# eth-ait/MultiPly

Hardware: NVIDIA H100
Metric: rays/sec (higher is better)
Workload: dtype f32 (fp16 hi/lo split tensor-core operands, fp32 accumulate)

## Files before the change

multiply_b200/csrc/mlp_tc.cu:

```cuda
#include "common.cuh"
#include <vector>
#include <mutex>
#include <type_traits>
#include <stdlib.h>

namespace mp {

enum {
  K_SP_PLAIN = 0,
  K_SP_SAVE = 1,
  K_SP_SEED = 2,
  K_FEAT = 3,
  K_BWD = 4,
  K_FINAL_GRAD = 5,
  K_RELU = 6
};
enum {
  F_INJECT_EMB = 1,
  F_SDF_DOT = 2,
  F_SKIP_GRAD = 4,
  F_EXTRA_IN = 8,
  F_RGB_OUT = 16
};
constexpr int kMaxSteps = 24;
constexpr int kSlotBytes = 32768;
constexpr int kRing = 3;

struct TcStep {
  int nk;
  int kind;
  int flags;
  int sig;
  const float* bias;
  int slot_off;
  int sc;
  int terms;
};

struct TcProgram {
  int nsteps;
  TcStep step[kMaxSteps];
  const uint4* blob;
  const float* inv_scale;
  int d_in, multires, E, inj_col, n_extra;
  const float* w8row;
  const float* b8;
  const float* Wrgb;
  const float* brgb;
};

struct TcIO : MlpCall {
  float rz;
  char* scratch;
  size_t scratch_per_cta;
  unsigned long long* stalls;
};

constexpr int kConsumers = 2;
constexpr int kThreads = 128 * (1 + kConsumers);

enum { PH_STEP = 0, PH_FULL = 1, PH_WGMMA = 2, PH_BAR = 3, PH_EPI = 4, PH_EMPTY = 5 };
constexpr int kStallWarps = 1 + 4 * kConsumers;
static_assert(MP_STALL_WARPS == kStallWarps && MP_STALL_KINDS == K_RELU + 1 && MP_STALL_PHASES == PH_EMPTY + 1 &&
                  MP_STALL_PROLOGUE == MP_STALL_KINDS * MP_STALL_PHASES && MP_STALL_ELAPSED == MP_STALL_PROLOGUE + 1 &&
                  MP_STALL_WORDS == MP_STALL_ELAPSED + 1,
              "stall record layout of include/multiply_b200.h");
template <bool PROF>
__device__ __forceinline__ long long stall_clock() {
  if constexpr (PROF) return clock64();
  else return 0;
}
__device__ __forceinline__ void stall_add(unsigned long long* rec, int word, long long clocks) {
  atomicAdd(rec + word, (unsigned long long)clocks);
}

constexpr size_t kSigBytes = (size_t)8 * kConsumers * 32 * 128 * 16;
constexpr size_t kFeatBytes = (size_t)kConsumers * 32 * 128 * 16;
constexpr size_t kGeBytes = (size_t)96 * 128 * 4;
constexpr size_t kEmbBytes = (size_t)96 * 128 * 4;
constexpr size_t kScratchPerCta = kSigBytes + kFeatBytes + kGeBytes + kEmbBytes;

constexpr int kAhead = 4;

constexpr int kABytes = 2 * 4 * 128 * 128;
constexpr int kSmemBytes = kABytes + kRing * kSlotBytes + 256 + 1024;
static_assert(kSmemBytes <= 232448, "shared memory budget of one CTA (227 KB)");

__device__ __forceinline__ uint32_t smem_u32(const void* p) { return (uint32_t)__cvta_generic_to_shared(p); }

__device__ __forceinline__ void mbar_init(uint64_t* bar, uint32_t count) {
  asm volatile("mbarrier.init.shared::cta.b64 [%0], %1;" ::"r"(smem_u32(bar)), "r"(count));
}
__device__ __forceinline__ void mbar_arrive(uint64_t* bar) {
  asm volatile("mbarrier.arrive.shared::cta.b64 _, [%0];" ::"r"(smem_u32(bar)) : "memory");
}
__device__ __forceinline__ void mbar_expect_tx(uint64_t* bar, uint32_t bytes) {
  asm volatile("mbarrier.arrive.expect_tx.shared::cta.b64 _, [%0], %1;" ::"r"(smem_u32(bar)), "r"(bytes) : "memory");
}
__device__ __forceinline__ void mbar_wait(uint64_t* bar, uint32_t parity) {
  asm volatile(
      "{\n"
      ".reg .pred p;\n"
      "WAIT_LOOP:\n"
      "mbarrier.try_wait.parity.shared::cta.b64 p, [%0], %1;\n"
      "@p bra WAIT_DONE;\n"
      "bra WAIT_LOOP;\n"
      "WAIT_DONE:\n"
      "}\n" ::"r"(smem_u32(bar)),
      "r"(parity)
      : "memory");
}
__device__ __forceinline__ void bulk_g2s(void* dst, const void* src, uint32_t bytes, uint64_t* bar) {
  asm volatile("cp.async.bulk.shared::cluster.global.mbarrier::complete_tx::bytes [%0], [%1], %2, [%3];" ::"r"(
                   smem_u32(dst)),
               "l"(src), "r"(bytes), "r"(smem_u32(bar))
               : "memory");
}
__device__ __forceinline__ void prefetch_l2(const void* p, uint32_t bytes) {
  asm volatile("cp.async.bulk.prefetch.L2.global [%0], %1;" ::"l"(p), "r"(bytes) : "memory");
}
__device__ __forceinline__ void fence_async_smem() { asm volatile("fence.proxy.async.shared::cta;" ::: "memory"); }

__device__ __forceinline__ void wg_sync(int id) { asm volatile("bar.sync %0, 128;" ::"r"(id) : "memory"); }

__device__ __forceinline__ void wgmma_fence() { asm volatile("wgmma.fence.sync.aligned;" ::: "memory"); }
__device__ __forceinline__ void wgmma_commit() { asm volatile("wgmma.commit_group.sync.aligned;" ::: "memory"); }
template <int N>
__device__ __forceinline__ void wgmma_wait() {
  asm volatile("wgmma.wait_group.sync.aligned %0;" ::"n"(N) : "memory");
}
__device__ __forceinline__ void acc_fence(float* d) {
#pragma unroll
  for (int i = 0; i < 128; ++i) asm volatile("" : "+f"(d[i])::"memory");
}

#define MP_D4(i) "+f"(d[i]), "+f"(d[i + 1]), "+f"(d[i + 2]), "+f"(d[i + 3])
#define MP_D16(i) MP_D4(i), MP_D4(i + 4), MP_D4(i + 8), MP_D4(i + 12)
__device__ __forceinline__ void wgmma_f16(float* d, uint64_t a_desc, uint64_t b_desc, uint32_t accumulate) {
  asm volatile(
      "{\n"
      ".reg .pred p;\n"
      "setp.ne.b32 p, %130, 0;\n"
      "wgmma.mma_async.sync.aligned.m64n256k16.f32.f16.f16 "
      "{%0, %1, %2, %3, %4, %5, %6, %7, %8, %9, %10, %11, %12, %13, %14, %15, "
      "%16, %17, %18, %19, %20, %21, %22, %23, %24, %25, %26, %27, %28, %29, %30, %31, "
      "%32, %33, %34, %35, %36, %37, %38, %39, %40, %41, %42, %43, %44, %45, %46, %47, "
      "%48, %49, %50, %51, %52, %53, %54, %55, %56, %57, %58, %59, %60, %61, %62, %63, "
      "%64, %65, %66, %67, %68, %69, %70, %71, %72, %73, %74, %75, %76, %77, %78, %79, "
      "%80, %81, %82, %83, %84, %85, %86, %87, %88, %89, %90, %91, %92, %93, %94, %95, "
      "%96, %97, %98, %99, %100, %101, %102, %103, %104, %105, %106, %107, %108, %109, %110, %111, "
      "%112, %113, %114, %115, %116, %117, %118, %119, %120, %121, %122, %123, %124, %125, %126, %127}, "
      "%128, %129, p, 1, 1, 0, 0;\n"
      "}\n"
      : MP_D16(0), MP_D16(16), MP_D16(32), MP_D16(48), MP_D16(64), MP_D16(80), MP_D16(96), MP_D16(112)
      : "l"(a_desc), "l"(b_desc), "r"(accumulate));
}
#undef MP_D16
#undef MP_D4

__device__ __forceinline__ uint64_t make_desc(uint32_t saddr) {
  return (uint64_t)((saddr >> 4) & 0x3FFF) | (1ull << 16) | ((uint64_t)(1024 >> 4) << 32) | (1ull << 62);
}

__device__ __forceinline__ uint32_t a_off(int row, int kb, int ch) {
  return (uint32_t)(kb * 16384 + row * 128 + ((ch ^ (row & 7)) << 4));
}

__device__ __forceinline__ void split2(float a, float b, uint32_t& hi, uint32_t& lo) {
  __half2 h = __floats2half2_rn(a, b);
  float2 f = __half22float2(h);
  __half2 l = __floats2half2_rn(a - f.x, b - f.y);
  hi = *(uint32_t*)&h;
  lo = *(uint32_t*)&l;
}
__device__ __forceinline__ void split8(const float* v, uint4& hi, uint4& lo) {
  split2(v[0], v[1], hi.x, lo.x);
  split2(v[2], v[3], hi.y, lo.y);
  split2(v[4], v[5], hi.z, lo.z);
  split2(v[6], v[7], hi.w, lo.w);
}

__device__ __forceinline__ void sts128(uint32_t A32, uint32_t off, const uint4& v) {
  asm volatile("st.shared.v4.b32 [%0], {%1, %2, %3, %4};" ::"r"(A32 + off), "r"(v.x), "r"(v.y), "r"(v.z), "r"(v.w));
}
__device__ __forceinline__ void store_a8(uint32_t A32, int row, int col, const float* v) {
  uint4 hi, lo;
  split8(v, hi, lo);
  uint32_t o = a_off(row, col >> 6, (col >> 3) & 7);
  sts128(A32, o, hi);
  sts128(A32, 65536 + o, lo);
}
__device__ __forceinline__ void stsm4(uint32_t addr, uint32_t a, uint32_t b, uint32_t c, uint32_t e) {
  asm volatile("stmatrix.sync.aligned.m8n8.x4.shared.b16 [%0], {%1, %2, %3, %4};" ::"r"(addr), "r"(a), "r"(b), "r"(c),
               "r"(e));
}
__device__ __forceinline__ void store_pairs(uint32_t lane_base, uint32_t lane_x, int jp, const uint4& hi, const uint4& lo) {
  const uint32_t addr = lane_base + (uint32_t)(jp >> 2) * 16384u + ((((uint32_t)(2 * jp) & 7u) ^ lane_x) << 4);
  stsm4(addr, hi.x, hi.y, hi.z, hi.w);
  stsm4(addr + 65536u, lo.x, lo.y, lo.z, lo.w);
}
__device__ __forceinline__ void store_acc16(uint32_t lane_base, uint32_t lane_x, int jp, const float* v) {
  uint4 hi, lo;
  split8(v, hi, lo);
  store_pairs(lane_base, lane_x, jp, hi, lo);
}

__device__ __forceinline__ float quad_sum(float v) {
  v += __shfl_xor_sync(0xffffffffu, v, 1);
  v += __shfl_xor_sync(0xffffffffu, v, 2);
  return v;
}

__device__ __forceinline__ float4 ld_stream(const float4* p) {
  float4 v;
  asm volatile("ld.global.cg.v4.f32 {%0,%1,%2,%3}, [%4];" : "=f"(v.x), "=f"(v.y), "=f"(v.z), "=f"(v.w) : "l"(p));
  return v;
}
__device__ __forceinline__ uint4 ld_stream(const uint4* p) {
  uint4 v;
  asm volatile("ld.global.cg.v4.u32 {%0,%1,%2,%3}, [%4];" : "=r"(v.x), "=r"(v.y), "=r"(v.z), "=r"(v.w) : "l"(p));
  return v;
}
__device__ __forceinline__ void st_stream(float4* p, const float4& v) {
  asm volatile("st.global.cg.v4.f32 [%0], {%1,%2,%3,%4};" ::"l"(p), "f"(v.x), "f"(v.y), "f"(v.z), "f"(v.w) : "memory");
}
__device__ __forceinline__ void st_stream(uint4* p, const uint4& v) {
  asm volatile("st.global.cg.v4.u32 [%0], {%1,%2,%3,%4};" ::"l"(p), "r"(v.x), "r"(v.y), "r"(v.z), "r"(v.w) : "memory");
}

__device__ __forceinline__ void discard_line(const void* p, float dep) {
  asm volatile("discard.global.L2 [%0], 128;" ::"l"(p), "f"(dep) : "memory");
}
__device__ __forceinline__ void discard_line(const void* p, uint32_t dep) {
  asm volatile("discard.global.L2 [%0], 128;" ::"l"(p), "r"(dep) : "memory");
}

__device__ __forceinline__ float ex2_approx(float x) {
  float y;
  asm("ex2.approx.ftz.f32 %0, %1;" : "=f"(y) : "f"(x));
  return y;
}
__device__ __forceinline__ float lg2_approx(float x) {
  float y;
  asm("lg2.approx.ftz.f32 %0, %1;" : "=f"(y) : "f"(x));
  return y;
}
__device__ __forceinline__ float rcp_approx(float x) {
  float y;
  asm("rcp.approx.ftz.f32 %0, %1;" : "=f"(y) : "f"(x));
  return y;
}
__device__ __forceinline__ float softplus_fast(float z) {
  float t = z * 144.26950408889634f;
  float u = ex2_approx(t);
  float y = lg2_approx(1.f + u) * 0.0069314718055994531f;
  return t > 28.853900817779268f ? z : y;
}
__device__ __forceinline__ void softplus_fast_grad(float z, float& y, float& d) {
  float t = z * 144.26950408889634f;
  float u = ex2_approx(t);
  float w = 1.f + u;
  float r = rcp_approx(w);
  float ys = lg2_approx(w) * 0.0069314718055994531f;
  bool big = t > 28.853900817779268f;
  y = big ? z : ys;
  d = big ? 1.f : u * r;
}

__device__ __forceinline__ void final_grad(const TcProgram& P, const TcIO& io, const float* acc, float isc, int q,
                                           const float* ge, const float* emb, const int (&rowt)[2],
                                           const bool (&valid)[2], const int (&pt)[2], const int (&slot)[2],
                                           float (&nrm)[2][3]) {
  const int d = P.d_in;
  float gax[2][4] = {{0.f, 0.f, 0.f, 0.f}, {0.f, 0.f, 0.f, 0.f}};
  const int nterm = 1 + 2 * P.multires;
#pragma unroll
  for (int j = 0; j < 8; ++j) {
    if (j < 2 * d) {
      const int a = j >> 1;
#pragma unroll
      for (int e = 0; e < 4; ++e) {
        const int jj = (8 * j + 2 * q + (e & 1)) & 15;
        if (jj < nterm) {
          const int h = e >> 1;
          const int fq = (jj - 1) >> 1;
          const bool is_cos = ((jj - 1) & 1) != 0;
          const int k = (jj == 0) ? a : d + 2 * fq * d + (is_cos ? d : 0) + a;
          const float pg = ge[(size_t)k * 128 + rowt[h]];
          const float tot = fmaf(acc[4 * j + e], isc, pg);
          float w = 1.f;
          if (jj > 0) {
            const float pe = emb[(size_t)(is_cos ? k - d : k + d) * 128 + rowt[h]];
            w = (float)(1 << fq) * (is_cos ? -pe : pe);
          }
          gax[h][a] = fmaf(w, tot, gax[h][a]);
        }
      }
    }
  }
#pragma unroll
  for (int h = 0; h < 2; ++h) {
#pragma unroll
    for (int a = 0; a < 4; ++a) gax[h][a] = quad_sum(gax[h][a]);
    const float gx0 = gax[h][0], gx1 = d > 1 ? gax[h][1] : 0.f, gx2 = d > 2 ? gax[h][2] : 0.f;
    if (q == 0 && io.grad && valid[h]) {
      io.grad[3 * (size_t)pt[h]] = gx0;
      io.grad[3 * (size_t)pt[h] + 1] = gx1;
      io.grad[3 * (size_t)pt[h] + 2] = gx2;
    }
    float n0 = 0.f, n1 = 0.f, n2 = 0.f;
    if (io.jinv && valid[h]) {
      const float4* J4 = (const float4*)(io.jinv + 12 * (size_t)pt[h]);
      const float4 ja = __ldg(J4), jb = __ldg(J4 + 1), jc = __ldg(J4 + 2);
      float v0 = gx0 * ja.x + gx1 * ja.w + gx2 * jb.z;
      float v1 = gx0 * ja.y + gx1 * jb.x + gx2 * jb.w;
      float v2 = gx0 * ja.z + gx1 * jb.y + gx2 * jc.x;
      float nr = fmaxf(sqrtf(v0 * v0 + v1 * v1 + v2 * v2), 1e-12f);
      const float inr = 1.f / nr;
      v0 *= inr; v1 *= inr; v2 *= inr;
      float n2r = fmaxf(sqrtf(v0 * v0 + v1 * v1 + v2 * v2), 1e-6f);
      const float in2 = 1.f / n2r;
      n0 = v0 * in2; n1 = v1 * in2; n2 = v2 * in2;
      if (q == 0 && io.nrm) {
        io.nrm[3 * (size_t)slot[h]] = n0;
        io.nrm[3 * (size_t)slot[h] + 1] = n1;
        io.nrm[3 * (size_t)slot[h] + 2] = n2;
      }
    }
    nrm[h][0] = n0;
    nrm[h][1] = n1;
    nrm[h][2] = n2;
  }
}

template <bool PROF>
__global__ void __launch_bounds__(kThreads, 1) tc_chain_kernel(const __grid_constant__ TcProgram P,
                                                               const __grid_constant__ TcIO io) {
  extern __shared__ uint8_t smem_raw[];
  const int warp = threadIdx.x >> 5, lane = threadIdx.x & 31;
  char* base = (char*)(((uintptr_t)smem_raw + 1023) & ~(uintptr_t)1023);
  char* A = base;
  const uint32_t A32 = smem_u32(A);
  char* ring = base + kABytes;
  uint64_t* bars = (uint64_t*)(ring + kRing * kSlotBytes);
  uint64_t* full = bars;
  uint64_t* empty = bars + kRing;

  const int count = io.count ? min(io.cap, *io.count) : io.cap;
  const int ntiles = (count + 127) >> 7;

  if (threadIdx.x == 0) {
    for (int i = 0; i < kRing; ++i) {
      mbar_init(&full[i], 1);
      mbar_init(&empty[i], 4 * kConsumers);
    }
    asm volatile("fence.mbarrier_init.release.cluster;" ::: "memory");
  }
  __syncthreads();

  if (warp < 4) {
    asm volatile("setmaxnreg.dec.sync.aligned.u32 40;\n" ::: "memory");
    if (warp == 0 && lane == 0) {
      const long long t_run = stall_clock<PROF>();
      uint32_t it = 0;
      for (int tile = blockIdx.x; tile < ntiles; tile += gridDim.x) {
        for (int s = 0; s < P.nsteps; ++s) {
          const long long t_step = stall_clock<PROF>();
          long long c_empty = 0;
          const char* src = (const char*)P.blob + (size_t)P.step[s].slot_off * kSlotBytes;
          const int nslot = 2 * P.step[s].nk;
          const int jstep = P.step[s].terms == 1 ? 2 : 1;
          for (int j = 0; j < nslot; j += jstep, ++it) {
            int r = it % kRing;
            uint32_t ph = (it / kRing) & 1;
            const long long t0 = stall_clock<PROF>();
            mbar_wait(&empty[r], ph ^ 1);
            c_empty += stall_clock<PROF>() - t0;
            mbar_expect_tx(&full[r], kSlotBytes);
            bulk_g2s(ring + (size_t)r * kSlotBytes, src + (size_t)j * kSlotBytes, kSlotBytes, &full[r]);
          }
          if constexpr (PROF) {
            unsigned long long* rec = io.stalls + (size_t)blockIdx.x * kStallWarps * MP_STALL_WORDS +
                                      P.step[s].kind * MP_STALL_PHASES;
            stall_add(rec, PH_STEP, clock64() - t_step);
            stall_add(rec, PH_EMPTY, c_empty);
          }
        }
      }
      if constexpr (PROF)
        stall_add(io.stalls + (size_t)blockIdx.x * kStallWarps * MP_STALL_WORDS, MP_STALL_ELAPSED, clock64() - t_run);
    }
    return;
  }
  asm volatile("setmaxnreg.inc.sync.aligned.u32 232;\n" ::: "memory");
  const long long t_run = stall_clock<PROF>();
  auto srec = [&]() { return io.stalls + ((size_t)blockIdx.x * kStallWarps + warp - 3) * MP_STALL_WORDS; };
  const int g = (warp >> 2) - 1;
  const int t = threadIdx.x & 127;
  const int wq = warp & 3, q = lane & 3;
  const int bar_id = 1 + g;
  int rowt[2];
  rowt[0] = 64 * g + 16 * wq + (lane >> 2);
  rowt[1] = rowt[0] + 8;
  const int mi = lane >> 3, rr = lane & 7;
  const uint32_t lane_base = A32 + (uint32_t)(64 * g + 16 * wq + 8 * (mi & 1) + rr) * 128u;
  const uint32_t lane_x = (uint32_t)((mi >> 1) ^ rr);
  const uint32_t a_hi = A32 + (uint32_t)g * 8192u, a_lo = a_hi + 65536u;

  char* scr = io.scratch + (size_t)blockIdx.x * io.scratch_per_cta;
  float4* sig = (float4*)scr;
  uint4* fsc = (uint4*)(scr + kSigBytes) + (size_t)g * 32 * 128;
  float* ge = (float*)(scr + kSigBytes + kFeatBytes);
  float* emb = (float*)(scr + kSigBytes + kFeatBytes + kGeBytes);
  const int d = P.d_in, E = P.E;

  float acc[128];
#pragma unroll
  for (int i = 0; i < 128; ++i) acc[i] = 0.f;
  uint32_t it = 0;

  for (int tile = blockIdx.x; tile < ntiles; tile += gridDim.x) {
    const long long t_tile = stall_clock<PROF>();
    int pt[2], slot[2];
    bool valid[2];
    float x[2][4];
#pragma unroll
    for (int h = 0; h < 2; ++h) {
      pt[h] = tile * 128 + rowt[h];
      valid[h] = pt[h] < count;
      for (int a = 0; a < 4; ++a) x[h][a] = 0.f;
      if (valid[h])
        for (int a = 0; a < d; ++a) x[h][a] = io.x[(size_t)pt[h] * d + a];
      slot[h] = valid[h] ? (io.slot ? io.slot[pt[h]] : pt[h]) : 0;
    }
    {
      const int npair = d * P.multires;
      for (int pi = q; pi < npair; pi += 4) {
        const int f = pi / d, a = pi - f * d;
#pragma unroll
        for (int h = 0; h < 2; ++h) {
          float sn, cs;
          sincosf(__fmul_rn(x[h][a], (float)(1 << f)), &sn, &cs);
          emb[(size_t)(d + 2 * f * d + a) * 128 + rowt[h]] = sn;
          emb[(size_t)(d + (2 * f + 1) * d + a) * 128 + rowt[h]] = cs;
        }
      }
      if (q == 0)
        for (int a = 0; a < d; ++a)
#pragma unroll
          for (int h = 0; h < 2; ++h) emb[(size_t)a * 128 + rowt[h]] = x[h][a];
      if (io.dirs) {
        float dv[2][3];
#pragma unroll
        for (int h = 0; h < 2; ++h)
          for (int a = 0; a < 3; ++a) dv[h][a] = valid[h] ? io.dirs[(size_t)pt[h] * 3 + a] : 0.f;
        const int nvp = (P.n_extra - 3) / 2;
        for (int pi = q; pi < nvp; pi += 4) {
          const int f = pi / 3, a = pi - f * 3;
#pragma unroll
          for (int h = 0; h < 2; ++h) {
            float sn, cs;
            sincosf(__fmul_rn(dv[h][a], (float)(1 << f)), &sn, &cs);
            ge[(size_t)(3 + 6 * f + a) * 128 + rowt[h]] = sn;
            ge[(size_t)(3 + 6 * f + 3 + a) * 128 + rowt[h]] = cs;
          }
        }
        if (q == 0)
          for (int a = 0; a < 3; ++a)
#pragma unroll
            for (int h = 0; h < 2; ++h) ge[(size_t)a * 128 + rowt[h]] = dv[h][a];
      }
      __threadfence_block();
      wg_sync(bar_id);
      const int njp = P.step[0].nk * 4;
      for (int jp = 0; jp < njp; ++jp) {
        float v[8];
#pragma unroll
        for (int i = 0; i < 8; ++i) {
          const int c = 16 * jp + 8 * (i >> 2) + 2 * q + (i & 1);
          v[i] = (c < E) ? emb[(size_t)c * 128 + rowt[(i >> 1) & 1]] : 0.f;
        }
        store_acc16(lane_base, lane_x, jp, v);
      }
    }
    float nrm[2][3] = {{0.f, 0.f, 0.f}, {0.f, 0.f, 0.f}};
    if constexpr (PROF)
      if (lane == 0) stall_add(srec(), MP_STALL_PROLOGUE, clock64() - t_tile);
    for (int s = 0; s < P.nsteps; ++s) {
      const TcStep st = P.step[s];
      const long long t_step = stall_clock<PROF>();
      long long c_full = 0, c_wgmma = 0, c_bar = 0;
      const float isc = P.inv_scale[st.sc] * fmaf(io.rz, (float)(4 * st.nk * (st.terms == 1 ? 1 : 3)), 1.f);
      const bool one_term = st.terms == 1;
      if (t == 0) {
        char* ws = io.scratch + (size_t)blockIdx.x * io.scratch_per_cta;
        if (st.kind == K_BWD && st.sig >= 0)
          prefetch_l2(ws + (((size_t)st.sig * kConsumers + g) * 32 * 128) * 16, 32 * 128 * 16);
        if (st.kind == K_FINAL_GRAD) prefetch_l2(ws + kSigBytes + (size_t)g * 32 * 128 * 16, 32 * 128 * 16);
      }

      fence_async_smem();
      {
        const long long t0 = stall_clock<PROF>();
        wg_sync(bar_id);
        c_bar += stall_clock<PROF>() - t0;
      }
      wgmma_fence();
      bool held = false;
      uint32_t held_slot = 0;
      auto release = [&](uint32_t slot_it) {
        if (lane == 0) mbar_arrive(&empty[slot_it % kRing]);
      };
      auto slot_issued = [&](uint32_t slot_it) {
        wgmma_commit();
        if (held) {
          const long long t0 = stall_clock<PROF>();
          wgmma_wait<1>();
          c_wgmma += stall_clock<PROF>() - t0;
          release(held_slot);
        }
        held = true;
        held_slot = slot_it;
      };
      for (int kc = 0; kc < st.nk; ++kc) {
        if (kc == 4) {
          {
            const long long t0 = stall_clock<PROF>();
            wgmma_wait<0>();
            acc_fence(acc);
            c_wgmma += stall_clock<PROF>() - t0;
          }
          if (held) release(held_slot);
          held = false;
#pragma unroll
          for (int h = 0; h < 2; ++h) {
#pragma unroll
            for (int c8 = 0; c8 < 16; c8 += 8) {
              const int e0 = 16 * q + c8;
              float xv[8];
#pragma unroll
              for (int j = 0; j < 8; ++j) xv[j] = 0.f;
              if (io.dirs) {
#pragma unroll
                for (int j = 0; j < 8; ++j)
                  if (e0 + j < P.n_extra) xv[j] = ge[(size_t)(e0 + j) * 128 + rowt[h]];
              } else if (e0 == 0) {
                xv[0] = x[h][0]; xv[1] = x[h][1]; xv[2] = x[h][2];
                xv[3] = nrm[h][0]; xv[4] = nrm[h][1]; xv[5] = nrm[h][2];
              }
              store_a8(A32, rowt[h], e0, xv);
            }
          }
          fence_async_smem();
          {
            const long long t0 = stall_clock<PROF>();
            wg_sync(bar_id);
            c_bar += stall_clock<PROF>() - t0;
          }
          wgmma_fence();
        }
        const uint32_t ka = (uint32_t)(kc & 3) * 16384u;
        int r = it % kRing;
        long long t0 = stall_clock<PROF>();
        mbar_wait(&full[r], (it / kRing) & 1);
        c_full += stall_clock<PROF>() - t0;
        uint32_t wb = smem_u32(ring + (size_t)r * kSlotBytes);
#pragma unroll
        for (int ks = 0; ks < 4; ++ks) {
          const uint64_t bd = make_desc(wb + ks * 32);
          wgmma_f16(acc, make_desc(a_hi + ka + ks * 32), bd, (kc | ks) != 0);
          if (!one_term) wgmma_f16(acc, make_desc(a_lo + ka + ks * 32), bd, 1);
        }
        slot_issued(it++);
        if (!one_term) {
          r = it % kRing;
          t0 = stall_clock<PROF>();
          mbar_wait(&full[r], (it / kRing) & 1);
          c_full += stall_clock<PROF>() - t0;
          wb = smem_u32(ring + (size_t)r * kSlotBytes);
#pragma unroll
          for (int ks = 0; ks < 4; ++ks) wgmma_f16(acc, make_desc(a_hi + ka + ks * 32), make_desc(wb + ks * 32), 1);
          slot_issued(it++);
        }
      }
      {
        const long long t0 = stall_clock<PROF>();
        wgmma_wait<0>();
        acc_fence(acc);
        c_wgmma += stall_clock<PROF>() - t0;
      }
      if (held) release(held_slot);

      const long long t_epi = stall_clock<PROF>();
      auto step_done = [&]() {
        if constexpr (PROF) {
          if (lane == 0) {
            const long long now = clock64();
            unsigned long long* rec = srec() + st.kind * MP_STALL_PHASES;
            stall_add(rec, PH_STEP, now - t_step);
            stall_add(rec, PH_FULL, c_full);
            stall_add(rec, PH_WGMMA, c_wgmma);
            stall_add(rec, PH_BAR, c_bar);
            stall_add(rec, PH_EPI, now - t_epi);
          }
        }
      };
      auto reload_features = [&]() {
        uint4 pre[kAhead][2];
#pragma unroll
        for (int k = 0; k < kAhead; ++k) {
          pre[k][0] = ld_stream(&fsc[(size_t)k * 128 + t]);
          pre[k][1] = ld_stream(&fsc[(size_t)(16 + k) * 128 + t]);
        }
#pragma unroll
        for (int jp = 0; jp < 16; ++jp) {
          const uint4 fh = pre[jp % kAhead][0];
          const uint4 fl = pre[jp % kAhead][1];
          if (jp + kAhead < 16) {
            pre[jp % kAhead][0] = ld_stream(&fsc[(size_t)(jp + kAhead) * 128 + t]);
            pre[jp % kAhead][1] = ld_stream(&fsc[(size_t)(16 + jp + kAhead) * 128 + t]);
          }
          store_pairs(lane_base, lane_x, jp, fh, fl);
          if ((lane & 7) == 0) {
            discard_line(&fsc[(size_t)jp * 128 + t], fh.x);
            discard_line(&fsc[(size_t)(16 + jp) * 128 + t], fl.x);
          }
        }
      };
      if (st.kind == K_FINAL_GRAD) {
        final_grad(P, io, acc, isc, q, ge, emb, rowt, valid, pt, slot, nrm);
        if (s + 1 < P.nsteps) reload_features();
        step_done();
        continue;
      }

      auto run_epi = [&](auto kind) {
        constexpr int KIND = decltype(kind)::value;
        float dot[2][3] = {{0.f, 0.f, 0.f}, {0.f, 0.f, 0.f}};
        const float4* sig_g = &sig[((size_t)(st.sig < 0 ? 0 : st.sig) * kConsumers + g) * 32 * 128 + t];
        float4 sig_pre[2 * kAhead];
        if constexpr (KIND == K_BWD) {
#pragma unroll
          for (int k = 0; k < 2 * kAhead; ++k)
            sig_pre[k] = st.sig >= 0 ? ld_stream(sig_g + (size_t)k * 128) : make_float4(1.f, 1.f, 1.f, 1.f);
        }
#pragma unroll
        for (int jp = 0; jp < 16; ++jp) {
          float* v = acc + 8 * jp;
          float yv[8];
#pragma unroll
          for (int jj = 0; jj < 2; ++jj) {
            const int j = 2 * jp + jj;
            const int c = 8 * j + 2 * q;
            float* u = v + 4 * jj;
            float b[2] = {0.f, 0.f};
            if constexpr (KIND != K_BWD) {
              const float2 b2 = __ldg((const float2*)(st.bias + c));
              b[0] = b2.x;
              b[1] = b2.y;
            }
            if constexpr (KIND == K_SP_SEED) {
              const float2 w2 = __ldg((const float2*)(P.w8row + c));
              const float w[2] = {w2.x, w2.y};
#pragma unroll
              for (int e = 0; e < 4; ++e) {
                float y, dd;
                softplus_fast_grad(fmaf(u[e], isc, b[e & 1]), y, dd);
                dot[e >> 1][0] = fmaf(y, w[e & 1], dot[e >> 1][0]);
                yv[4 * jj + e] = y;
                u[e] = dd * w[e & 1];
              }
            } else if constexpr (KIND == K_SP_SAVE || KIND == K_SP_PLAIN) {
              if constexpr (KIND == K_SP_SAVE) {
                float dd[4];
#pragma unroll
                for (int e = 0; e < 4; ++e) softplus_fast_grad(fmaf(u[e], isc, b[e & 1]), u[e], dd[e]);
                st_stream(&sig[(((size_t)st.sig * kConsumers + g) * 32 + j) * 128 + t], make_float4(dd[0], dd[1], dd[2], dd[3]));
              } else {
#pragma unroll
                for (int e = 0; e < 4; ++e) u[e] = softplus_fast(fmaf(u[e], isc, b[e & 1]));
              }
              if ((st.flags & F_INJECT_EMB) && c + 1 >= P.inj_col) {
#pragma unroll
                for (int e = 0; e < 4; ++e)
                  if (c + (e & 1) >= P.inj_col) u[e] = emb[(size_t)(c + (e & 1) - P.inj_col) * 128 + rowt[e >> 1]];
              }
              if (st.flags & F_SDF_DOT) {
                const float2 w2 = __ldg((const float2*)(P.w8row + c));
                dot[0][0] = fmaf(u[0], w2.x, fmaf(u[1], w2.y, dot[0][0]));
                dot[1][0] = fmaf(u[2], w2.x, fmaf(u[3], w2.y, dot[1][0]));
              }
            } else if constexpr (KIND == K_FEAT) {
#pragma unroll
              for (int e = 0; e < 4; ++e) u[e] = fmaf(u[e], isc, b[e & 1]);
              if (io.feat) {
#pragma unroll
                for (int h = 0; h < 2; ++h)
                  if (valid[h]) *(float2*)(io.feat + (size_t)pt[h] * 256 + c) = make_float2(u[2 * h], u[2 * h + 1]);
              }
            } else if constexpr (KIND == K_BWD) {
              const float4 s4 = sig_pre[j % (2 * kAhead)];
              if (j + 2 * kAhead < 32 && st.sig >= 0)
                sig_pre[j % (2 * kAhead)] = ld_stream(sig_g + (size_t)(j + 2 * kAhead) * 128);
              const float4* sp = sig_g + (size_t)j * 128;
              const float sv[4] = {s4.x, s4.y, s4.z, s4.w};
              if ((st.flags & F_SKIP_GRAD) && c + 1 >= P.inj_col) {
#pragma unroll
                for (int e = 0; e < 4; ++e) {
                  const float gval = u[e] * isc;
                  const int col = c + (e & 1);
                  if (col >= P.inj_col) {
                    ge[(size_t)(col - P.inj_col) * 128 + rowt[e >> 1]] = gval;
                    u[e] = 0.f;
                  } else {
                    u[e] = gval * sv[e];
                  }
                }
              } else {
#pragma unroll
                for (int e = 0; e < 4; ++e) u[e] *= isc * sv[e];
              }
              if (st.sig >= 0 && (lane & 7) == 0) discard_line(sp, s4.x);
            } else {
#pragma unroll
              for (int e = 0; e < 4; ++e) u[e] = fmaxf(fmaf(u[e], isc, b[e & 1]), 0.f);
              if (st.flags & F_RGB_OUT) {
#pragma unroll
                for (int k = 0; k < 3; ++k) {
                  const float2 w2 = __ldg((const float2*)(P.Wrgb + 256 * k + c));
                  dot[0][k] = fmaf(u[0], w2.x, fmaf(u[1], w2.y, dot[0][k]));
                  dot[1][k] = fmaf(u[2], w2.x, fmaf(u[3], w2.y, dot[1][k]));
                }
              }
            }
          }
          if constexpr (KIND == K_SP_SEED) {
            uint4 fh, fl;
            split8(yv, fh, fl);
            st_stream(&fsc[(size_t)jp * 128 + t], fh);
            st_stream(&fsc[(size_t)(16 + jp) * 128 + t], fl);
          }
          bool to_a = true;
          if constexpr (KIND == K_RELU) to_a = !(st.flags & F_RGB_OUT);
          if (to_a) store_acc16(lane_base, lane_x, jp, v);
        }
        if (st.flags & F_SDF_DOT) {
#pragma unroll
          for (int h = 0; h < 2; ++h) {
            const float sdot = quad_sum(dot[h][0]);
            if (q == 0 && valid[h] && io.sdf) io.sdf[slot[h]] = __ldg(P.b8) + sdot;
          }
        }
        if constexpr (KIND == K_RELU) {
          if (st.flags & F_RGB_OUT) {
#pragma unroll
            for (int h = 0; h < 2; ++h) {
#pragma unroll
              for (int k = 0; k < 3; ++k) {
                const float z = __ldg(P.brgb + k) + quad_sum(dot[h][k]);
                if (q == 0 && valid[h] && io.rgb) io.rgb[3 * (size_t)slot[h] + k] = 1.f / (1.f + __expf(-z));
              }
            }
          }
        }
      };
      switch (st.kind) {
        case K_SP_PLAIN: run_epi(std::integral_constant<int, K_SP_PLAIN>{}); break;
        case K_SP_SAVE: run_epi(std::integral_constant<int, K_SP_SAVE>{}); break;
        case K_SP_SEED: run_epi(std::integral_constant<int, K_SP_SEED>{}); break;
        case K_FEAT: run_epi(std::integral_constant<int, K_FEAT>{}); break;
        case K_BWD: run_epi(std::integral_constant<int, K_BWD>{}); break;
        default: run_epi(std::integral_constant<int, K_RELU>{}); break;
      }
      if (st.flags & F_SKIP_GRAD) __threadfence_block();
      step_done();
    }
  }
  if constexpr (PROF)
    if (lane == 0) stall_add(srec(), MP_STALL_ELAPSED, clock64() - t_run);
}

struct TcSrc {
  const float* W;
  int ld, transposed, n_off, n_valid, k_valid, nk, total, perm16, slot_off;
};

constexpr int kLdM = 320;

struct TcBlob {
  TcProgram sdf_prog;
  TcProgram full_prog;
  TcProgram fwd_prog;
  float* Mfold;
  float* w8row;
  float* Wrgb;
  float* b8feat;
  float* inv_scale;
  uint8_t* blob;
  std::vector<TcSrc> src;
};

__global__ void absmax_kernel(const float* __restrict__ W, int n, float* __restrict__ inv_scale) {
  __shared__ float s[256];
  float m = 0.f;
  for (int i = threadIdx.x; i < n; i += blockDim.x) m = fmaxf(m, fabsf(W[i]));
  s[threadIdx.x] = m;
  __syncthreads();
  for (int o = 128; o > 0; o >>= 1) {
    if (threadIdx.x < o) s[threadIdx.x] = fmaxf(s[threadIdx.x], s[threadIdx.x + o]);
    __syncthreads();
  }
  if (threadIdx.x == 0) {
    float mx = s[0];
    int ex = 0;
    if (mx > 0.f) frexpf(mx, &ex);
    float sc = ldexpf(1.f, 14 - ex);
    inv_scale[0] = 1.f / sc;
  }
}

__global__ void pack_slot_kernel(const float* __restrict__ W, int ld, int transposed, int n_off, int k_off,
                                 int n_valid, int k_valid, int kc, const float* __restrict__ inv_scale,
                                 uint8_t* __restrict__ dst_hi, uint8_t* __restrict__ dst_lo, int perm16) {
  int idx = blockIdx.x * blockDim.x + threadIdx.x;
  if (idx >= 256 * 64) return;
  int n = idx >> 6, k = idx & 63;
  int kk = kc * 64 + k;
  int ns = n;
  if (perm16) {
    const int dd = perm16, a = n >> 4, j = n & 15;
    ns = n_valid;
    if (n < 64 && a < dd) {
      const int k = (j == 0) ? a : dd + ((j - 1) >> 1) * 2 * dd + ((j - 1) & 1) * dd + a;
      if (k < n_valid) ns = k;
    }
  }
  float w = 0.f;
  if (ns < n_valid && kk < k_valid)
    w = transposed ? W[(size_t)(k_off + kk) * ld + n_off + ns] : W[(size_t)(n_off + ns) * ld + k_off + kk];
  w = __fdiv_rn(w, inv_scale[0]);
  __half h = __float2half_rn(w);
  __half l = __float2half_rn(w - __half2float(h));
  uint32_t off = (uint32_t)(n * 128 + ((((k >> 3) ^ (n & 7))) << 4) + (k & 7) * 2);
  *(__half*)(dst_hi + off) = h;
  *(__half*)(dst_lo + off) = l;
}

__global__ void fold_mm_kernel(const float* __restrict__ Wc, int ldc, int coff, const float* __restrict__ W8f, int ld8,
                               const float* __restrict__ b8f, int n_rows, float* __restrict__ M, int ldm,
                               float* __restrict__ cb) {
  int k = blockIdx.x * 16 + threadIdx.x, n = blockIdx.y * 16 + threadIdx.y;
  if (n >= n_rows || k >= 256) return;
  const float* w = Wc + (size_t)n * ldc + coff;
  double acc = 0.0;
  for (int j = 0; j < 256; ++j) acc += (double)w[j] * (double)W8f[(size_t)j * ld8 + k];
  M[(size_t)n * ldm + k] = (float)acc;
  if (k == 0) {
    double a2 = 0.0;
    for (int j = 0; j < 256; ++j) a2 += (double)w[j] * (double)b8f[j];
    cb[n] = (float)a2;
  }
}

__global__ void fill_extra_cols_kernel(const float* __restrict__ Wt, int n_out, int n_extra, float* __restrict__ M, int ldm) {
  int i = blockIdx.x * blockDim.x + threadIdx.x;
  if (i >= 256 * 64) return;
  int n = i >> 6, e = i & 63;
  M[(size_t)n * ldm + 256 + e] = (n < n_out && e < n_extra) ? Wt[(size_t)e * n_out + n] : 0.f;
}

TcBlob* tc_new() { return new TcBlob(); }
void tc_free(TcBlob* tb) { delete tb; }

static int tc_programs(const Field& f, TcBlob& tb) {
  int nslots = 0;
  auto layer = [&](TcStep& stp, int kind, int flags, int sig, const float* bias, const float* W, int ld, int transposed,
                   int n_off, int n_valid, int k_valid, int nk, int total, int perm16 = 0) {
    stp = TcStep{nk, kind, flags, sig, bias, nslots, (int)tb.src.size(), 3};
    tb.src.push_back(TcSrc{W, ld, transposed, n_off, n_valid, k_valid, nk, total, perm16, nslots});
    nslots += 2 * nk;
  };
  const int E = f.emb_dim;
  TcProgram P{};
  P.d_in = f.d_in;
  P.multires = f.multires;
  P.E = E;
  P.inj_col = kHidden - E;
  P.w8row = tb.w8row;
  P.b8 = f.imp_b[8];
  P.Wrgb = tb.Wrgb;
  P.n_extra = f.ren_extra;
  int s = 0;
  for (int l = 0; l < 8; ++l) {
    const int in = f.imp_in[l], out = f.imp_out[l];
    const int flags = ((l == f.skip_layer - 1) ? F_INJECT_EMB : 0) | ((l == 7) ? F_SDF_DOT : 0);
    layer(P.step[s++], K_SP_PLAIN, flags, l, (l == 0) ? f.imp_b0_eff : f.imp_b[l], f.imp_W[l], in, 0, 0, out,
          (l == 0) ? E : in, (l == 0) ? (E + 63) / 64 : 4, out * in);
  }
  P.nsteps = s;
  tb.sdf_prog = P;
  tb.fwd_prog = P;
  layer(tb.fwd_prog.step[s], K_FEAT, 0, -1, tb.b8feat, f.imp_W[8], 256, 0, 1, 256, 256, 4, 257 * 256);
  tb.fwd_prog.nsteps = s + 1;
  if (f.tc_full && f.ren_mode == 1) {
    layer(P.step[s++], K_RELU, F_EXTRA_IN | F_RGB_OUT, -1, f.ren_b0_fold, tb.Mfold, kLdM, 0, 0, f.ren_out[0], kLdM, 5,
          256 * kLdM);
    P.brgb = f.ren_b[1];
    P.nsteps = s;
    tb.full_prog = P;
  }
  if (f.tc_full && f.ren_mode == 0) {
    for (int l = 0; l < 8; ++l) P.step[l].kind = (l == 7) ? K_SP_SEED : K_SP_SAVE;
    for (int l = 7; l >= 1; --l) {
      const int in = f.imp_in[l], out = f.imp_out[l];
      layer(P.step[s++], K_BWD, (l == f.skip_layer) ? F_SKIP_GRAD : 0, l - 1, nullptr, f.imp_W[l], in, 1, 0, in, out, 4,
            out * in);
    }
    layer(P.step[s++], K_FINAL_GRAD, 0, -1, nullptr, f.imp_W[0], f.imp_in[0], 1, 0, E, 256, 4, 256 * f.imp_in[0],
          f.d_in);
    layer(P.step[s++], K_RELU, F_EXTRA_IN, -1, f.ren_b0_fold, tb.Mfold, kLdM, 0, 0, 256, kLdM, 5, 256 * kLdM);
    for (int l = 1; l < 4; ++l)
      layer(P.step[s++], K_RELU, (l == 3) ? F_RGB_OUT : 0, -1, f.ren_b[l], f.ren_W[l], 256, 0, 0, 256, 256, 4,
            256 * 256);
    P.brgb = f.ren_b[4];
    P.nsteps = s;
// ... 253 lines not shown
```

Before: 483,300.

## Specialize epilogue on flags, prefetch constants, and split first-MMA zero-init

Specializes the epilogue at compile time on the step's flags (SDF dot, RGB output). Bias, w8 and RGB weight constants are now software-prefetched a few column pairs ahead, and the epilogue processes two column pairs per pass with the sigma stores deferred. The first wgmma of each step uses a scale-d=0 variant instead of a runtime predicate, which removes the per-tile accumulator zeroing. It also drops the memory clobber on streaming stores, and moves embedding injection into a separate scalar pass that writes half-precision hi/lo values into the A tile. The cost is more template instantiations, added register pressure from the prefetched constants, and an extra workgroup sync plus 16-bit shared stores for the injection.

```diff
diff --git a/multiply_b200/csrc/mlp_tc.cu b/multiply_b200/csrc/mlp_tc.cu
--- a/multiply_b200/csrc/mlp_tc.cu
+++ b/multiply_b200/csrc/mlp_tc.cu
@@ -81,6 +81,8 @@
 constexpr size_t kScratchPerCta = kSigBytes + kFeatBytes + kGeBytes + kEmbBytes;
 
 constexpr int kAhead = 4;
+constexpr int kEpiW = 2;
+constexpr int kCAhead = 3;
 
 constexpr int kABytes = 2 * 4 * 128 * 128;
 constexpr int kSmemBytes = kABytes + kRing * kSlotBytes + 256 + 1024;
@@ -136,11 +138,8 @@
 
 #define MP_D4(i) "+f"(d[i]), "+f"(d[i + 1]), "+f"(d[i + 2]), "+f"(d[i + 3])
 #define MP_D16(i) MP_D4(i), MP_D4(i + 4), MP_D4(i + 8), MP_D4(i + 12)
-__device__ __forceinline__ void wgmma_f16(float* d, uint64_t a_desc, uint64_t b_desc, uint32_t accumulate) {
+__device__ __forceinline__ void wgmma_f16(float* d, uint64_t a_desc, uint64_t b_desc) {
   asm volatile(
-      "{\n"
-      ".reg .pred p;\n"
-      "setp.ne.b32 p, %130, 0;\n"
       "wgmma.mma_async.sync.aligned.m64n256k16.f32.f16.f16 "
       "{%0, %1, %2, %3, %4, %5, %6, %7, %8, %9, %10, %11, %12, %13, %14, %15, "
       "%16, %17, %18, %19, %20, %21, %22, %23, %24, %25, %26, %27, %28, %29, %30, %31, "
@@ -150,10 +149,28 @@
       "%80, %81, %82, %83, %84, %85, %86, %87, %88, %89, %90, %91, %92, %93, %94, %95, "
       "%96, %97, %98, %99, %100, %101, %102, %103, %104, %105, %106, %107, %108, %109, %110, %111, "
       "%112, %113, %114, %115, %116, %117, %118, %119, %120, %121, %122, %123, %124, %125, %126, %127}, "
-      "%128, %129, p, 1, 1, 0, 0;\n"
-      "}\n"
+      "%128, %129, 1, 1, 1, 0, 0;\n"
       : MP_D16(0), MP_D16(16), MP_D16(32), MP_D16(48), MP_D16(64), MP_D16(80), MP_D16(96), MP_D16(112)
-      : "l"(a_desc), "l"(b_desc), "r"(accumulate));
+      : "l"(a_desc), "l"(b_desc));
+}
+#undef MP_D16
+#undef MP_D4
+#define MP_D4(i) "=f"(d[i]), "=f"(d[i + 1]), "=f"(d[i + 2]), "=f"(d[i + 3])
+#define MP_D16(i) MP_D4(i), MP_D4(i + 4), MP_D4(i + 8), MP_D4(i + 12)
+__device__ __forceinline__ void wgmma_f16_first(float* d, uint64_t a_desc, uint64_t b_desc) {
+  asm volatile(
+      "wgmma.mma_async.sync.aligned.m64n256k16.f32.f16.f16 "
+      "{%0, %1, %2, %3, %4, %5, %6, %7, %8, %9, %10, %11, %12, %13, %14, %15, "
+      "%16, %17, %18, %19, %20, %21, %22, %23, %24, %25, %26, %27, %28, %29, %30, %31, "
+      "%32, %33, %34, %35, %36, %37, %38, %39, %40, %41, %42, %43, %44, %45, %46, %47, "
+      "%48, %49, %50, %51, %52, %53, %54, %55, %56, %57, %58, %59, %60, %61, %62, %63, "
+      "%64, %65, %66, %67, %68, %69, %70, %71, %72, %73, %74, %75, %76, %77, %78, %79, "
+      "%80, %81, %82, %83, %84, %85, %86, %87, %88, %89, %90, %91, %92, %93, %94, %95, "
+      "%96, %97, %98, %99, %100, %101, %102, %103, %104, %105, %106, %107, %108, %109, %110, %111, "
+      "%112, %113, %114, %115, %116, %117, %118, %119, %120, %121, %122, %123, %124, %125, %126, %127}, "
+      "%128, %129, 0, 1, 1, 0, 0;\n"
+      : MP_D16(0), MP_D16(16), MP_D16(32), MP_D16(48), MP_D16(64), MP_D16(80), MP_D16(96), MP_D16(112)
+      : "l"(a_desc), "l"(b_desc));
 }
 #undef MP_D16
 #undef MP_D4
@@ -183,6 +200,9 @@
 __device__ __forceinline__ void sts128(uint32_t A32, uint32_t off, const uint4& v) {
   asm volatile("st.shared.v4.b32 [%0], {%1, %2, %3, %4};" ::"r"(A32 + off), "r"(v.x), "r"(v.y), "r"(v.z), "r"(v.w));
 }
+__device__ __forceinline__ void sts16(uint32_t A32, uint32_t off, __half v) {
+  asm volatile("st.shared.b16 [%0], %1;" ::"r"(A32 + off), "h"(__half_as_ushort(v)));
+}
 __device__ __forceinline__ void store_a8(uint32_t A32, int row, int col, const float* v) {
   uint4 hi, lo;
   split8(v, hi, lo);
@@ -205,6 +225,19 @@
   store_pairs(lane_base, lane_x, jp, hi, lo);
 }
 
+template <int V>
+using IntC = std::integral_constant<int, V>;
+template <int MASK, int FL = 0, class F>
+__device__ __forceinline__ void with_flags(int flags, F&& f) {
+  if constexpr (MASK == 0) {
+    f(IntC<FL>{});
+  } else {
+    constexpr int bit = MASK & -MASK;
+    if (flags & bit) with_flags<MASK & ~bit, FL | bit>(flags, f);
+    else with_flags<MASK & ~bit, FL>(flags, f);
+  }
+}
+
 __device__ __forceinline__ float quad_sum(float v) {
   v += __shfl_xor_sync(0xffffffffu, v, 1);
   v += __shfl_xor_sync(0xffffffffu, v, 2);
@@ -222,10 +255,10 @@
   return v;
 }
 __device__ __forceinline__ void st_stream(float4* p, const float4& v) {
-  asm volatile("st.global.cg.v4.f32 [%0], {%1,%2,%3,%4};" ::"l"(p), "f"(v.x), "f"(v.y), "f"(v.z), "f"(v.w) : "memory");
+  asm volatile("st.global.cg.v4.f32 [%0], {%1,%2,%3,%4};" ::"l"(p), "f"(v.x), "f"(v.y), "f"(v.z), "f"(v.w));
 }
 __device__ __forceinline__ void st_stream(uint4* p, const uint4& v) {
-  asm volatile("st.global.cg.v4.u32 [%0], {%1,%2,%3,%4};" ::"l"(p), "r"(v.x), "r"(v.y), "r"(v.z), "r"(v.w) : "memory");
+  asm volatile("st.global.cg.v4.u32 [%0], {%1,%2,%3,%4};" ::"l"(p), "r"(v.x), "r"(v.y), "r"(v.z), "r"(v.w));
 }
 
 __device__ __forceinline__ void discard_line(const void* p, float dep) {
@@ -415,8 +448,6 @@
   const int d = P.d_in, E = P.E;
 
   float acc[128];
-#pragma unroll
-  for (int i = 0; i < 128; ++i) acc[i] = 0.f;
   uint32_t it = 0;
 
   for (int tile = blockIdx.x; tile < ntiles; tile += gridDim.x) {
@@ -491,7 +522,6 @@
       const long long t_step = stall_clock<PROF>();
       long long c_full = 0, c_wgmma = 0, c_bar = 0;
       const float isc = P.inv_scale[st.sc] * fmaf(io.rz, (float)(4 * st.nk * (st.terms == 1 ? 1 : 3)), 1.f);
-      const bool one_term = st.terms == 1;
       if (t == 0) {
         char* ws = io.scratch + (size_t)blockIdx.x * io.scratch_per_cta;
         if (st.kind == K_BWD && st.sig >= 0)
@@ -522,8 +552,9 @@
         held = true;
         held_slot = slot_it;
       };
-      for (int kc = 0; kc < st.nk; ++kc) {
-        if (kc == 4) {
+      auto chunk = [&](int kc, auto first, auto one) {
+        constexpr bool FIRST = decltype(first)::value, ONE_TERM = decltype(one)::value;
+        if (!FIRST && kc == 4) {
           {
             const long long t0 = stall_clock<PROF>();
             wgmma_wait<0>();
@@ -568,21 +599,28 @@
 #pragma unroll
         for (int ks = 0; ks < 4; ++ks) {
           const uint64_t bd = make_desc(wb + ks * 32);
-          wgmma_f16(acc, make_desc(a_hi + ka + ks * 32), bd, (kc | ks) != 0);
-          if (!one_term) wgmma_f16(acc, make_desc(a_lo + ka + ks * 32), bd, 1);
+          if (FIRST && ks == 0) wgmma_f16_first(acc, make_desc(a_hi + ka + ks * 32), bd);
+          else wgmma_f16(acc, make_desc(a_hi + ka + ks * 32), bd);
+          if constexpr (!ONE_TERM) wgmma_f16(acc, make_desc(a_lo + ka + ks * 32), bd);
         }
         slot_issued(it++);
-        if (!one_term) {
+        if constexpr (!ONE_TERM) {
           r = it % kRing;
           t0 = stall_clock<PROF>();
           mbar_wait(&full[r], (it / kRing) & 1);
           c_full += stall_clock<PROF>() - t0;
           wb = smem_u32(ring + (size_t)r * kSlotBytes);
 #pragma unroll
-          for (int ks = 0; ks < 4; ++ks) wgmma_f16(acc, make_desc(a_hi + ka + ks * 32), make_desc(wb + ks * 32), 1);
+          for (int ks = 0; ks < 4; ++ks) wgmma_f16(acc, make_desc(a_hi + ka + ks * 32), make_desc(wb + ks * 32));
           slot_issued(it++);
         }
-      }
+      };
+      auto mmas = [&](auto one) {
+        chunk(0, std::true_type{}, one);
+        for (int kc = 1; kc < st.nk; ++kc) chunk(kc, std::false_type{}, one);
+      };
+      if (st.terms == 1) mmas(std::true_type{});
+      else mmas(std::false_type{});
       {
         const long long t0 = stall_clock<PROF>();
         wgmma_wait<0>();
@@ -634,9 +672,32 @@
         continue;
       }
 
-      auto run_epi = [&](auto kind) {
+      auto run_epi = [&](auto kind, auto flags) {
         constexpr int KIND = decltype(kind)::value;
+        constexpr int FL = decltype(flags)::value;
+        constexpr bool kBias = KIND != K_BWD;
+        constexpr bool kW8 = KIND == K_SP_SEED || (FL & F_SDF_DOT) != 0;
+        constexpr bool kRgb = KIND == K_RELU && (FL & F_RGB_OUT) != 0;
+        constexpr int W = KIND == K_BWD ? 1 : kEpiW;
         float dot[2][3] = {{0.f, 0.f, 0.f}, {0.f, 0.f, 0.f}};
+        struct Consts {
+          float2 b[2], w8[2], rgb[2][3];
+        };
+        auto load_consts = [&](int jp, Consts& k) {
+#pragma unroll
+          for (int jj = 0; jj < 2; ++jj) {
+            const int c = 16 * jp + 8 * jj + 2 * q;
+            if constexpr (kBias) k.b[jj] = __ldg((const float2*)(st.bias + c));
+            if constexpr (kW8) k.w8[jj] = __ldg((const float2*)(P.w8row + c));
+            if constexpr (kRgb) {
+#pragma unroll
+              for (int kk = 0; kk < 3; ++kk) k.rgb[jj][kk] = __ldg((const float2*)(P.Wrgb + 256 * kk + c));
+            }
+          }
+        };
+        Consts cpre[kCAhead];
+#pragma unroll
+        for (int k = 0; k < kCAhead; ++k) load_consts(k, cpre[k]);
         const float4* sig_g = &sig[((size_t)(st.sig < 0 ? 0 : st.sig) * kConsumers + g) * 32 * 128 + t];
         float4 sig_pre[2 * kAhead];
         if constexpr (KIND == K_BWD) {
@@ -645,132 +706,154 @@
             sig_pre[k] = st.sig >= 0 ? ld_stream(sig_g + (size_t)k * 128) : make_float4(1.f, 1.f, 1.f, 1.f);
         }
 #pragma unroll
-        for (int jp = 0; jp < 16; ++jp) {
-          float* v = acc + 8 * jp;
-          float yv[8];
-#pragma unroll
-          for (int jj = 0; jj < 2; ++jj) {
-            const int j = 2 * jp + jj;
-            const int c = 8 * j + 2 * q;
-            float* u = v + 4 * jj;
-            float b[2] = {0.f, 0.f};
-            if constexpr (KIND != K_BWD) {
-              const float2 b2 = __ldg((const float2*)(st.bias + c));
-              b[0] = b2.x;
-              b[1] = b2.y;
-            }
-            if constexpr (KIND == K_SP_SEED) {
-              const float2 w2 = __ldg((const float2*)(P.w8row + c));
-              const float w[2] = {w2.x, w2.y};
-#pragma unroll
-              for (int e = 0; e < 4; ++e) {
-                float y, dd;
-                softplus_fast_grad(fmaf(u[e], isc, b[e & 1]), y, dd);
-                dot[e >> 1][0] = fmaf(y, w[e & 1], dot[e >> 1][0]);
-                yv[4 * jj + e] = y;
-                u[e] = dd * w[e & 1];
+        for (int jp0 = 0; jp0 < 16; jp0 += W) {
+          float dsv[W][2][4];
+          float yv[W][8];
+#pragma unroll
+          for (int wi = 0; wi < W; ++wi) {
+            const int jp = jp0 + wi;
+            float* v = acc + 8 * jp;
+            const Consts cs = cpre[jp % kCAhead];
+            if (jp + kCAhead < 16) load_consts(jp + kCAhead, cpre[jp % kCAhead]);
+#pragma unroll
+            for (int jj = 0; jj < 2; ++jj) {
+              const int j = 2 * jp + jj;
+              const int c = 8 * j + 2 * q;
+              float* u = v + 4 * jj;
+              float b[2] = {0.f, 0.f};
+              if constexpr (kBias) {
+                b[0] = cs.b[jj].x;
+                b[1] = cs.b[jj].y;
               }
-            } else if constexpr (KIND == K_SP_SAVE || KIND == K_SP_PLAIN) {
-              if constexpr (KIND == K_SP_SAVE) {
-                float dd[4];
-#pragma unroll
-                for (int e = 0; e < 4; ++e) softplus_fast_grad(fmaf(u[e], isc, b[e & 1]), u[e], dd[e]);
-                st_stream(&sig[(((size_t)st.sig * kConsumers + g) * 32 + j) * 128 + t], make_float4(dd[0], dd[1], dd[2], dd[3]));
+              if constexpr (KIND == K_SP_SEED) {
+                const float w[2] = {cs.w8[jj].x, cs.w8[jj].y};
+#pragma unroll
+                for (int e = 0; e < 4; ++e) {
+                  float y, dd;
+                  softplus_fast_grad(fmaf(u[e], isc, b[e & 1]), y, dd);
+                  dot[e >> 1][0] = fmaf(y, w[e & 1], dot[e >> 1][0]);
+                  yv[wi][4 * jj + e] = y;
+                  u[e] = dd * w[e & 1];
+                }
+              } else if constexpr (KIND == K_SP_SAVE || KIND == K_SP_PLAIN) {
+                if constexpr (KIND == K_SP_SAVE) {
+#pragma unroll
+                  for (int e = 0; e < 4; ++e) softplus_fast_grad(fmaf(u[e], isc, b[e & 1]), u[e], dsv[wi][jj][e]);
+                } else {
+#pragma unroll
+                  for (int e = 0; e < 4; ++e) u[e] = softplus_fast(fmaf(u[e], isc, b[e & 1]));
+                }
+                if constexpr ((FL & F_SDF_DOT) != 0) {
+                  const float2 w2 = cs.w8[jj];
+                  dot[0][0] = fmaf(u[0], w2.x, fmaf(u[1], w2.y, dot[0][0]));
+                  dot[1][0] = fmaf(u[2], w2.x, fmaf(u[3], w2.y, dot[1][0]));
+                }
+              } else if constexpr (KIND == K_FEAT) {
+#pragma unroll
+                for (int e = 0; e < 4; ++e) u[e] = fmaf(u[e], isc, b[e & 1]);
+                if (io.feat) {
+#pragma unroll
+                  for (int h = 0; h < 2; ++h)
+                    if (valid[h]) *(float2*)(io.feat + (size_t)pt[h] * 256 + c) = make_float2(u[2 * h], u[2 * h + 1]);
+                }
+              } else if constexpr (KIND == K_BWD) {
+                const float4 s4 = sig_pre[j % (2 * kAhead)];
+                if (j + 2 * kAhead < 32 && st.sig >= 0)
+                  sig_pre[j % (2 * kAhead)] = ld_stream(sig_g + (size_t)(j + 2 * kAhead) * 128);
+                const float4* sp = sig_g + (size_t)j * 128;
+                const float sv[4] = {s4.x, s4.y, s4.z, s4.w};
+                if ((st.flags & F_SKIP_GRAD) && c + 1 >= P.inj_col) {
+#pragma unroll
+                  for (int e = 0; e < 4; ++e) {
+                    const float gval = u[e] * isc;
+                    const int col = c + (e & 1);
+                    if (col >= P.inj_col) {
+                      ge[(size_t)(col - P.inj_col) * 128 + rowt[e >> 1]] = gval;
+                      u[e] = 0.f;
+                    } else {
+                      u[e] = gval * sv[e];
+                    }
+                  }
+                } else {
+#pragma unroll
+                  for (int e = 0; e < 4; ++e) u[e] *= isc * sv[e];
+                }
+                if (st.sig >= 0 && (lane & 7) == 0) discard_line(sp, s4.x);
               } else {
 #pragma unroll
-                for (int e = 0; e < 4; ++e) u[e] = softplus_fast(fmaf(u[e], isc, b[e & 1]));
-              }
-              if ((st.flags & F_INJECT_EMB) && c + 1 >= P.inj_col) {
-#pragma unroll
-                for (int e = 0; e < 4; ++e)
-                  if (c + (e & 1) >= P.inj_col) u[e] = emb[(size_t)(c + (e & 1) - P.inj_col) * 128 + rowt[e >> 1]];
-              }
-              if (st.flags & F_SDF_DOT) {
-                const float2 w2 = __ldg((const float2*)(P.w8row + c));
-                dot[0][0] = fmaf(u[0], w2.x, fmaf(u[1], w2.y, dot[0][0]));
-                dot[1][0] = fmaf(u[2], w2.x, fmaf(u[3], w2.y, dot[1][0]));
-              }
-            } else if constexpr (KIND == K_FEAT) {
-#pragma unroll
-              for (int e = 0; e < 4; ++e) u[e] = fmaf(u[e], isc, b[e & 1]);
-              if (io.feat) {
-#pragma unroll
-                for (int h = 0; h < 2; ++h)
-                  if (valid[h]) *(float2*)(io.feat + (size_t)pt[h] * 256 + c) = make_float2(u[2 * h], u[2 * h + 1]);
-              }
-            } else if constexpr (KIND == K_BWD) {
-              const float4 s4 = sig_pre[j % (2 * kAhead)];
-              if (j + 2 * kAhead < 32 && st.sig >= 0)
-                sig_pre[j % (2 * kAhead)] = ld_stream(sig_g + (size_t)(j + 2 * kAhead) * 128);
-              const float4* sp = sig_g + (size_t)j * 128;
-              const float sv[4] = {s4.x, s4.y, s4.z, s4.w};
-              if ((st.flags & F_SKIP_GRAD) && c + 1 >= P.inj_col) {
-#pragma unroll
-                for (int e = 0; e < 4; ++e) {
-                  const float gval = u[e] * isc;
-                  const int col = c + (e & 1);
-                  if (col >= P.inj_col) {
-                    ge[(size_t)(col - P.inj_col) * 128 + rowt[e >> 1]] = gval;
-                    u[e] = 0.f;
-                  } else {
-                    u[e] = gval * sv[e];
+                for (int e = 0; e < 4; ++e) u[e] = fmaxf(fmaf(u[e], isc, b[e & 1]), 0.f);
+                if constexpr (kRgb) {
+#pragma unroll
+                  for (int k = 0; k < 3; ++k) {
+                    const float2 w2 = cs.rgb[jj][k];
+                    dot[0][k] = fmaf(u[0], w2.x, fmaf(u[1], w2.y, dot[0][k]));
+                    dot[1][k] = fmaf(u[2], w2.x, fmaf(u[3], w2.y, dot[1][k]));
                   }
-                }
-              } else {
-#pragma unroll
-                for (int e = 0; e < 4; ++e) u[e] *= isc * sv[e];
-              }
-              if (st.sig >= 0 && (lane & 7) == 0) discard_line(sp, s4.x);
-            } else {
-#pragma unroll
-              for (int e = 0; e < 4; ++e) u[e] = fmaxf(fmaf(u[e], isc, b[e & 1]), 0.f);
-              if (st.flags & F_RGB_OUT) {
-#pragma unroll
-                for (int k = 0; k < 3; ++k) {
-                  const float2 w2 = __ldg((const float2*)(P.Wrgb + 256 * k + c));
-                  dot[0][k] = fmaf(u[0], w2.x, fmaf(u[1], w2.y, dot[0][k]));
-                  dot[1][k] = fmaf(u[2], w2.x, fmaf(u[3], w2.y, dot[1][k]));
                 }
               }
             }
           }
-          if constexpr (KIND == K_SP_SEED) {
-            uint4 fh, fl;
-            split8(yv, fh, fl);
-            st_stream(&fsc[(size_t)jp * 128 + t], fh);
-            st_stream(&fsc[(size_t)(16 + jp) * 128 + t], fl);
-          }
-          bool to_a = true;
-          if constexpr (KIND == K_RELU) to_a = !(st.flags & F_RGB_OUT);
-          if (to_a) store_acc16(lane_base, lane_x, jp, v);
-        }
-        if (st.flags & F_SDF_DOT) {
+#pragma unroll
+          for (int wi = 0; wi < W; ++wi) {
+            const int jp = jp0 + wi;
+            if constexpr (KIND == K_SP_SAVE) {
+#pragma unroll
+              for (int jj = 0; jj < 2; ++jj)
+                st_stream(&sig[(((size_t)st.sig * kConsumers + g) * 32 + 2 * jp + jj) * 128 + t],
+                          make_float4(dsv[wi][jj][0], dsv[wi][jj][1], dsv[wi][jj][2], dsv[wi][jj][3]));
+            }
+            if constexpr (KIND == K_SP_SEED) {
+              uint4 fh, fl;
+              split8(yv[wi], fh, fl);
+              st_stream(&fsc[(size_t)jp * 128 + t], fh);
+              st_stream(&fsc[(size_t)(16 + jp) * 128 + t], fl);
+            }
+            if constexpr (!kRgb) store_acc16(lane_base, lane_x, jp, acc + 8 * jp);
+          }
+        }
+        if (kW8 && (st.flags & F_SDF_DOT)) {
 #pragma unroll
           for (int h = 0; h < 2; ++h) {
             const float sdot = quad_sum(dot[h][0]);
             if (q == 0 && valid[h] && io.sdf) io.sdf[slot[h]] = __ldg(P.b8) + sdot;
           }
         }
-        if constexpr (KIND == K_RELU) {
-          if (st.flags & F_RGB_OUT) {
-#pragma unroll
-            for (int h = 0; h < 2; ++h) {
-#pragma unroll
-              for (int k = 0; k < 3; ++k) {
-                const float z = __ldg(P.brgb + k) + quad_sum(dot[h][k]);
-                if (q == 0 && valid[h] && io.rgb) io.rgb[3 * (size_t)slot[h] + k] = 1.f / (1.f + __expf(-z));
-              }
+        if constexpr (kRgb) {
+#pragma unroll
+          for (int h = 0; h < 2; ++h) {
+#pragma unroll
+            for (int k = 0; k < 3; ++k) {
+              const float z = __ldg(P.brgb + k) + quad_sum(dot[h][k]);
+              if (q == 0 && valid[h] && io.rgb) io.rgb[3 * (size_t)slot[h] + k] = 1.f / (1.f + __expf(-z));
             }
           }
+        }
+      };
+      auto inject_emb = [&]() {
+        wg_sync(bar_id);
+        const int row = 64 * g + (t >> 1);
+        for (int col = P.inj_col + (t & 1); col < kHidden; col += 2) {
+          const float v = emb[(size_t)(col - P.inj_col) * 128 + row];
+          const __half h = __float2half_rn(v);
+          const __half l = __float2half_rn(v - __half2float(h));
+          const uint32_t o = a_off(row, col >> 6, (col >> 3) & 7) + 2u * (uint32_t)(col & 7);
+          sts16(A32, o, h);
+          sts16(A32, 65536u + o, l);
         }
       };
       switch (st.kind) {
-        case K_SP_PLAIN: run_epi(std::integral_constant<int, K_SP_PLAIN>{}); break;
-        case K_SP_SAVE: run_epi(std::integral_constant<int, K_SP_SAVE>{}); break;
-        case K_SP_SEED: run_epi(std::integral_constant<int, K_SP_SEED>{}); break;
-        case K_FEAT: run_epi(std::integral_constant<int, K_FEAT>{}); break;
-        case K_BWD: run_epi(std::integral_constant<int, K_BWD>{}); break;
-        default: run_epi(std::integral_constant<int, K_RELU>{}); break;
+        case K_SP_PLAIN:
+          with_flags<F_SDF_DOT>(st.flags, [&](auto fl) { run_epi(IntC<K_SP_PLAIN>{}, fl); });
+          if (st.flags & F_INJECT_EMB) inject_emb();
+          break;
+        case K_SP_SAVE:
+          with_flags<F_SDF_DOT>(st.flags, [&](auto fl) { run_epi(IntC<K_SP_SAVE>{}, fl); });
+          if (st.flags & F_INJECT_EMB) inject_emb();
+          break;
+        case K_SP_SEED: run_epi(IntC<K_SP_SEED>{}, IntC<0>{}); break;
+        case K_FEAT: run_epi(IntC<K_FEAT>{}, IntC<0>{}); break;
+        case K_BWD: run_epi(IntC<K_BWD>{}, IntC<0>{}); break;
+        default: with_flags<F_RGB_OUT>(st.flags, [&](auto fl) { run_epi(IntC<K_RELU>{}, fl); }); break;
       }
       if (st.flags & F_SKIP_GRAD) __threadfence_block();
       step_done();
```

Result: faster. 515,600, median of 6 (+6.7%).
